# Sandy4321/dist-svgd

Measured on AMD Instinct MI355X. Metric: SVGD particle-updates/sec (n=65536,d=256) at 1/2/4/8 GPUs + % MFMA/HBM roofline, higher is better.
Workload: dtype f32; 1 GPU; dist-logreg DistSampler all_scores, Jacobi, median bandwidth; n=65536, d=256, N_global=16384, parallelism=dp1, particles_per_gpu=65536

## Files before the change

### dist-svgd_amd/csrc/phi_w1.hpp

```cpp
#pragma once
#include "gemm_x3.hpp"

namespace dsvgd {

struct PhiW1 {
  static constexpr int kThreads = 256;
  static constexpr int BM = 128, BC = 512, BJ = 16, P = 2;
  static constexpr int SA = P * BM * 32;
  static constexpr int kSmemBytes = 2 * SA;
  static constexpr int kScrLd = 44;
  static constexpr int kScrBytes = 16 * kScrLd * 4;
};

constexpr int kW1Sgb = 4;
__device__ __forceinline__ f32x4 w1_load(__amdgpu_buffer_rsrc_t r, int voff, int soff) {
  return __builtin_bit_cast(f32x4, __builtin_amdgcn_raw_buffer_load_b128(r, voff, soff, 0));
}
__device__ __forceinline__ f32x4 w1_load_nt(__amdgpu_buffer_rsrc_t r, int voff, int soff) {
  return __builtin_bit_cast(f32x4, __builtin_amdgcn_raw_buffer_load_b128(r, voff, soff, 2));
}

constexpr int w1_waves(int NI, bool EXP) { return NI == 2 && EXP ? 2 : 1; }
template <int DS, int NI = 4, bool EXP = true, int FAM = kFamRBF, class... PW>
__global__ __launch_bounds__(256)
__attribute__((amdgpu_waves_per_eu(w1_waves(NI, EXP), w1_waves(NI, EXP)))) void phi_w1_kernel(
    const float* A, int64_t a_npad, const _Float16* Yx, int64_t ldy,
    int64_t K, int64_t kchunk, const dsvgd_select_state* __restrict__ st, float* __restrict__ C,
    int64_t ldc, float* __restrict__ rowsum, int64_t m, int64_t row0, int sym,
    const float* __restrict__ colinv, int slice0, const float* __restrict__ gate, int gate_on,
    int ks_begin = 0, int ks_wrap = 0, int tcol0 = 0, int t_per = 0, int t_first = 0,
    int t_nblk = 1, int64_t t_ostride = 0, PW... pw_) {
  static_assert(sizeof...(PW) == (FAM == kFamIMQ ? 1 : 0), "pw: the IMQ instantiations only");
  [[maybe_unused]] const float pw = (0.f + ... + pw_);
  static_assert(NI == 4 || NI == 2, "NI: 4 or 2 column tiles per wave");
  static_assert(EXP || DS == 0, "the identity form is DS 0 only");
  const bool want_rs = EXP || rowsum != nullptr;
  if (gate && ((*gate != 0.f) != (gate_on != 0))) return;
  using F = FmtH2;
  constexpr int BC = 4 * 32 * NI;
  using V8 = F::V8;
  constexpr int P = PhiW1::P;
  constexpr bool TRK = DS == 1 || DS == 3 || DS == 4;
  __shared__ __attribute__((aligned(16))) char smem[PhiW1::kSmemBytes + (TRK ? 4 * PhiW1::kScrBytes : 0)];
  const int t = threadIdx.x, lane = t & 63, r = lane & 31, h = lane >> 5;
  const int w = __builtin_amdgcn_readfirstlane(t >> 6);
  const int64_t lin = (int64_t)blockIdx.z * gridDim.y + blockIdx.y;
  const bool xm = ((DS == 4 || DS == 0) && t_per == 1) || (DS == 3 && t_per > 0 && tcol0 == 1);
  const int64_t lid = lin * gridDim.x + blockIdx.x;
  const int64_t xu = (lid >> 3) * (8 / gridDim.z) + (lid & 7) / gridDim.z;
  const int64_t cbx = xm ? xu % gridDim.x : blockIdx.x;
  const int64_t by = xm ? xu / gridDim.x
                   : DS == 2 ? lin / gridDim.z
                   : DS == 1 ? (int64_t)gridDim.y - 1 - lin / gridDim.z : blockIdx.y;
  const int64_t bz = xm ? (lid & 7) % gridDim.z
                   : (DS == 1 || DS == 2) ? lin % gridDim.z : blockIdx.z;
  const bool tb = DS == 3 && t_per > 0;
  const int64_t tpart = tb ? by / t_per : 0;
  const int64_t byl = tb ? by % t_per : by;
  const int64_t i0 = byl * PhiW1::BM;
  const int64_t c0 = cbx * BC + w * 32 * NI;
  const int64_t kb0 = bz * kchunk, kend = min(K, kb0 + kchunk);
  int ks0 = (int)(kb0 / PhiW1::BJ) + (DS == 0 ? ks_begin : 0);
  int nsteps = kend > kb0 ? (int)((kend - kb0) / PhiW1::BJ) : 0;
  const int Z = (int)gridDim.z;
  const int kdir = DS == 2 ? -Z : DS == 1 ? Z : 1;
  auto wrapk = [&](int ks) { return (DS == 0 && ks_wrap > 0 && ks >= ks_wrap) ? ks - ks_wrap : ks; };
  const int kyoff = DS == 3 ? ks_begin : 0;
  if (DS == 2) {
    const int T = (int)((K - i0) / PhiW1::BJ);
    ks0 = (int)(K / PhiW1::BJ) - 1 - (int)bz;
    nsteps = T > bz ? (T - (int)bz + Z - 1) / Z : 0;
  } else if (DS == 1) {
    const int T = (int)(i0 / PhiW1::BJ);
    ks0 = (int)bz;
    nsteps = T > bz ? (T - (int)bz + Z - 1) / Z : 0;
  }
  const int ksp = DS == 4 ? (int)min(max(kb0, i0), kend) / PhiW1::BJ : 0;
  if (tb) {
    const int64_t at = ((int64_t)bz * (gridDim.y / t_per) + tpart) * t_ostride;
    C += at;
    rowsum += at;
  } else {
    C += (int64_t)(slice0 + bz) * m * ldc;
    rowsum += (int64_t)(slice0 + bz) * roundup128(m);
  }
  const float scale = !EXP ? 0.f : FAM == kFamIMQ ? st->inv_h : -st->inv_h * kLog2e;

  const __amdgpu_buffer_rsrc_t rD = __builtin_amdgcn_make_buffer_rsrc(
      (void*)(A + (i0 >> 7) * (a_npad >> 4) * kPanelElems), (short)0, 0x7fffffff, 0x00020000);
  const __amdgpu_buffer_rsrc_t rB =
      __builtin_amdgcn_make_buffer_rsrc((void*)(Yx + c0 * 16), (short)0, 0x7fffffff, 0x00020000);
  const int pstride = (int)(ldy * 32);
  const int vB = x3_off(r, h);
  const int vD = t * 32;
  const int srow = t >> 1, shalf = t & 1;
  const int aoff = x3_off(srow, shalf);
  auto diag0 = [&](int kfirst) {
    int64_t dg = row0 + i0 + srow - 8 * shalf - (int64_t)kfirst * PhiW1::BJ;
    if (DS == 0 && ks_wrap > 0 && row0 + i0 + srow < (int64_t)ks_begin * PhiW1::BJ)
      dg += (int64_t)ks_wrap * PhiW1::BJ;
    return (int)max(min(dg, (int64_t)(1 << 30)), (int64_t)-(1 << 30));
  };

  f32x16 acc[4][NI];
#pragma unroll
  for (int mi = 0; mi < 4; ++mi)
#pragma unroll
    for (int ni = 0; ni < NI; ++ni)
#pragma unroll
      for (int q = 0; q < 16; ++q) acc[mi][ni][q] = 0.f;
  float rs = 0.f;

  const int symI = tb ? (int)(((t_first + tpart) % t_nblk) * t_per + byl)
                   : DS == 3 ? tcol0 + (int)by : (sym || DS == 4) ? (int)(i0 >> 7) : -1;
  const int64_t pcols = a_npad >> 4;
  const int vP = (t >> 5) * kPanelElems * 4 + (t & 31) * 32;
  float* const scr = reinterpret_cast<float*>(smem + PhiW1::kSmemBytes + w * PhiW1::kScrBytes);
  const int sw_off = ((lane & 31) >> 1) * PhiW1::kScrLd + 16 * (lane >> 5) + 8 * (lane & 1);
  const int sr_off = 8 * shalf * PhiW1::kScrLd + (lane >> 1);

  auto phase = [&](auto TR_, const int ks0, const int nsteps, const int qd0) {
    constexpr bool TR = decltype(TR_)::value;
    if (nsteps <= 0) return;
    V8 b[NI][P];
    f32x4 dr[4][2];
    f32x4 tr[2];
    const int last = nsteps - 1;
    auto loadB = [&](int ni, int k) {
      const int soff = (wrapk(ks0 + kdir * min(k, last)) + kyoff) * P * pstride;
#pragma unroll
      for (int p = 0; p < P; ++p)
        b[ni][p] = __builtin_bit_cast(V8, w1_load(rB, vB + ni * 1024, soff + p * pstride));
    };
    auto loadD = [&](f32x4 (&d)[2], int k) {
      const int kc = min(k, last);
      const int64_t j0 = (int64_t)wrapk(ks0 + kdir * kc) * PhiW1::BJ;
      if constexpr (TR) {
        const float* src = A + (((j0 >> 7) * pcols + symI * 8) * kPanelElems + (j0 & 127) * 16);
        const __amdgpu_buffer_rsrc_t rT =
            __builtin_amdgcn_make_buffer_rsrc((void*)src, (short)0, 0x7fffffff, 0x00020000);
        d[0] = w1_load_nt(rT, vP, 0);
        d[1] = w1_load_nt(rT, vP + 16, 0);
      } else {
        const int soff = (int)(j0 >> 4) * kPanelElems * 4;
        d[0] = w1_load_nt(rD, vD, soff);
        d[1] = w1_load_nt(rD, vD + 16, soff);
      }
    };
    auto transpose = [&](const f32x4 (&d)[2], f32x4 (&o)[2]) {
      *reinterpret_cast<f32x4*>(scr + sw_off) = d[0];
      *reinterpret_cast<f32x4*>(scr + sw_off + 4) = d[1];
#pragma unroll
      for (int q = 0; q < 8; ++q) o[q >> 2][q & 3] = scr[sr_off + q * PhiW1::kScrLd];
    };
    auto stage = [&](char* st_, const f32x4 (&d)[2], int k) {
      const int qd = max(min(qd0 - kdir * k * PhiW1::BJ, 8), -1);
      float e[8];
#pragma unroll
      for (int q = 0; q < 8; ++q) {
        const float v = q < 4 ? d[0][q] : d[1][q - 4];
        const float x = !EXP ? v * F::kAScale
                        : FAM == kFamIMQ ? imq_pow(v, scale, pw, F::kAScaleLog2)
                                         : __builtin_amdgcn_exp2f(fmaf(v, scale, F::kAScaleLog2));
        e[q] = (EXP && !TR && qd == q) ? 0.f : x;
      }
      const float s = ((e[0] + e[1]) + (e[2] + e[3])) + ((e[4] + e[5]) + (e[6] + e[7]));
      rs += k <= last ? s : 0.f;
      V8 p0, p1;
#pragma unroll
      for (int q = 0; q < 8; ++q) {
        const _Float16 a0 = (_Float16)e[q];
        p0[q] = a0;
        p1[q] = (_Float16)(e[q] - (float)a0);
      }
      *reinterpret_cast<V8*>(st_ + aoff) = p0;
      *reinterpret_cast<V8*>(st_ + PhiW1::BM * 32 + aoff) = p1;
    };
    auto barrier = []() { asm volatile("s_waitcnt lgkmcnt(0)\n\ts_barrier" ::: "memory"); };
    auto step = [&](int k, const char* cur, char* nxt, const f32x4 (&ds_)[2], f32x4 (&dl)[2],
                    const f32x4 (&dt)[2]) {
      V8 a[4][P];
#pragma unroll
      for (int mi = 0; mi < 4; ++mi)
#pragma unroll
        for (int p = 0; p < P; ++p)
          a[mi][p] = *reinterpret_cast<const V8*>(cur + p * PhiW1::BM * 32 + x3_off(mi * 32 + r, h));
      if constexpr (TR)
        stage(nxt, tr, k + 1);
      else
        stage(nxt, ds_, k + 1);
#pragma unroll
      for (int ni = 0; ni < NI; ++ni) {
#pragma unroll
        for (int mi = 0; mi < 4; ++mi) acc[mi][ni] = mfma_fmt<F>(a[mi][1], b[ni][0], acc[mi][ni]);
#pragma unroll
        for (int mi = 0; mi < 4; ++mi) acc[mi][ni] = mfma_fmt<F>(a[mi][0], b[ni][1], acc[mi][ni]);
#pragma unroll
        for (int mi = 0; mi < 4; ++mi) acc[mi][ni] = mfma_fmt<F>(a[mi][0], b[ni][0], acc[mi][ni]);
        loadB(ni, k + 1);
      }
      if constexpr (TR) transpose(dt, tr);
      __builtin_amdgcn_sched_group_barrier(0x100, 8, 0);
#pragma unroll
      for (int i = 0; i < 4 * NI; ++i) {
        __builtin_amdgcn_sched_group_barrier(0x008, 1, 0);
        __builtin_amdgcn_sched_group_barrier(0x002, kW1Sgb, 0);
      }
      __builtin_amdgcn_sched_group_barrier(0x200, 2, 0);
#pragma unroll
      for (int i = 0; i < 8 * NI; ++i) {
        __builtin_amdgcn_sched_group_barrier(0x008, 1, 0);
        if (TR && i == 1) __builtin_amdgcn_sched_group_barrier(0x200, 2, 0);
        if (TR && i >= 2 && i < 10) __builtin_amdgcn_sched_group_barrier(0x100, 1, 0);
        if (i % 4 == 3) __builtin_amdgcn_sched_group_barrier(0x020, 1, 0);
      }
      loadD(dl, k + 3);
    };

#pragma unroll
    for (int ni = 0; ni < NI; ++ni) loadB(ni, 0);
    loadD(dr[0], 0);
    loadD(dr[1], 1);
    loadD(dr[2], 2);
    if constexpr (TR) {
      transpose(dr[0], tr);
      stage(smem, tr, 0);
      transpose(dr[1], tr);
    } else {
      stage(smem, dr[0], 0);
    }
    barrier();
    for (int k = 0; k < nsteps; k += 8) {
      step(k, smem, smem + PhiW1::SA, dr[1], dr[3], dr[2]);
      barrier();
      if (k + 1 >= nsteps) break;
      step(k + 1, smem + PhiW1::SA, smem, dr[2], dr[0], dr[3]);
      barrier();
      if (k + 2 >= nsteps) break;
      step(k + 2, smem, smem + PhiW1::SA, dr[3], dr[1], dr[0]);
      barrier();
      if (k + 3 >= nsteps) break;
      step(k + 3, smem + PhiW1::SA, smem, dr[0], dr[2], dr[1]);
      barrier();
      if (k + 4 >= nsteps) break;
      step(k + 4, smem, smem + PhiW1::SA, dr[1], dr[3], dr[2]);
      barrier();
      if (k + 5 >= nsteps) break;
      step(k + 5, smem + PhiW1::SA, smem, dr[2], dr[0], dr[3]);
      barrier();
      if (k + 6 >= nsteps) break;
      step(k + 6, smem, smem + PhiW1::SA, dr[3], dr[1], dr[0]);
      barrier();
      if (k + 7 >= nsteps) break;
      step(k + 7, smem + PhiW1::SA, smem, dr[0], dr[2], dr[1]);
      barrier();
    }
  };
  if constexpr (DS == 4) {
    phase(std::true_type{}, ks0, ksp - ks0, 0);
    phase(std::false_type{}, ksp, ks0 + nsteps - ksp, diag0(ksp));
  } else {
    phase(std::integral_constant<bool, DS == 1 || DS == 3>{}, ks0, nsteps, diag0(ks0));
  }

#pragma unroll
  for (int mi = 0; mi < 4; ++mi)
#pragma unroll
    for (int ni = 0; ni < NI; ++ni) {
      const int64_t col = c0 + ni * 32 + r;
      const float cs = colinv[col] * (1.f / F::kAScale);
#pragma unroll
      for (int q = 0; q < 16; ++q) {
        const int64_t row = i0 + mi * 32 + c_row(q, lane);
        if (row < m) C[row * ldc + col] = acc[mi][ni][q] * cs;
      }
    }
  {
    const float v = rs + __shfl_xor(rs, 1, 64);
    if (want_rs && cbx == 0 && shalf == 0 && i0 + srow < m)
      rowsum[i0 + srow] = v * (1.f / F::kAScale);
  }
}

}
```

Measured before the change: 4.817 million particle-updates/s.

## Split W1 K-loop into diagonal and plain phases, reschedule MFMA interleave

Splits the non-transposed K-loop into three phases so the per-element diagonal-zeroing check runs only on steps that overlap the diagonal block. Off-diagonal steps skip that compare. The change also rewrites the sched_group_barrier interleave into one loop that mixes in transcendental ops for the 2-wave variant, and simplifies the transposed-load address math with a precomputed base and scalar offsets. It disables packed-fp32 ops for the kernel. The extra phase instantiations increase code size and register pressure, and the diagonal-range math is a new source of correctness risk.

```diff
diff --git a/dist-svgd_amd/csrc/phi_w1.hpp b/dist-svgd_amd/csrc/phi_w1.hpp
--- a/dist-svgd_amd/csrc/phi_w1.hpp
+++ b/dist-svgd_amd/csrc/phi_w1.hpp
@@ -13,6 +13,8 @@
 };
 
 constexpr int kW1Sgb = 4;
+constexpr int kW1Mfv = 16;
+constexpr int kW1Exp = 8;
 __device__ __forceinline__ f32x4 w1_load(__amdgpu_buffer_rsrc_t r, int voff, int soff) {
   return __builtin_bit_cast(f32x4, __builtin_amdgcn_raw_buffer_load_b128(r, voff, soff, 0));
 }
@@ -21,6 +23,9 @@
 }
 
 constexpr int w1_waves(int NI, bool EXP) { return NI == 2 && EXP ? 2 : 1; }
+#if defined(__HIP_DEVICE_COMPILE__)
+#pragma clang attribute push(__attribute__((target("no-packed-fp32-ops"))), apply_to = function)
+#endif
 template <int DS, int NI = 4, bool EXP = true, int FAM = kFamRBF, class... PW>
 __global__ __launch_bounds__(256)
 __attribute__((amdgpu_waves_per_eu(w1_waves(NI, EXP), w1_waves(NI, EXP)))) void phi_w1_kernel(
@@ -75,7 +80,7 @@
     ks0 = (int)bz;
     nsteps = T > bz ? (T - (int)bz + Z - 1) / Z : 0;
   }
-  const int ksp = DS == 4 ? (int)min(max(kb0, i0), kend) / PhiW1::BJ : 0;
+  const int ksp = DS == 4 ? max((int)min(max(kb0, i0), kend) / PhiW1::BJ, ks0) : 0;
   if (tb) {
     const int64_t at = ((int64_t)bz * (gridDim.y / t_per) + tpart) * t_ostride;
     C += at;
@@ -119,8 +124,15 @@
   const int sw_off = ((lane & 31) >> 1) * PhiW1::kScrLd + 16 * (lane >> 5) + 8 * (lane & 1);
   const int sr_off = 8 * shalf * PhiW1::kScrLd + (lane >> 1);
 
-  auto phase = [&](auto TR_, const int ks0, const int nsteps, const int qd0) {
+  const char* const tbase = reinterpret_cast<const char*>(A + (int64_t)symI * 8 * kPanelElems);
+  const uint32_t trow = (uint32_t)(pcols * kPanelElems * 4);
+
+  auto phase = [&](auto TR_, auto DG_, auto U_, const int ks0, const int nsteps,
+                   const int qd0) __attribute__((always_inline)) {
     constexpr bool TR = decltype(TR_)::value;
+    constexpr bool DG = decltype(DG_)::value;
+    constexpr int U = decltype(U_)::value;
+    static_assert(!(TR && DG) && (U == 4 || U == 8), "phase: TR or DG; 4 or 8 K-steps per trip");
     if (nsteps <= 0) return;
     V8 b[NI][P];
     f32x4 dr[4][2];
@@ -133,16 +145,15 @@
         b[ni][p] = __builtin_bit_cast(V8, w1_load(rB, vB + ni * 1024, soff + p * pstride));
     };
     auto loadD = [&](f32x4 (&d)[2], int k) {
-      const int kc = min(k, last);
-      const int64_t j0 = (int64_t)wrapk(ks0 + kdir * kc) * PhiW1::BJ;
+      const int ks = wrapk(ks0 + kdir * min(k, last));
       if constexpr (TR) {
-        const float* src = A + (((j0 >> 7) * pcols + symI * 8) * kPanelElems + (j0 & 127) * 16);
-        const __amdgpu_buffer_rsrc_t rT =
-            __builtin_amdgcn_make_buffer_rsrc((void*)src, (short)0, 0x7fffffff, 0x00020000);
-        d[0] = w1_load_nt(rT, vP, 0);
-        d[1] = w1_load_nt(rT, vP + 16, 0);
+        const __amdgpu_buffer_rsrc_t rT = __builtin_amdgcn_make_buffer_rsrc(
+            (void*)(tbase + (uint64_t)(uint32_t)(ks >> 3) * trow), (short)0, 0x7fffffff, 0x00020000);
+        const int soff = (ks & 7) * (PhiW1::BJ * 16 * 4);
+        d[0] = w1_load_nt(rT, vP, soff);
+        d[1] = w1_load_nt(rT, vP + 16, soff);
       } else {
-        const int soff = (int)(j0 >> 4) * kPanelElems * 4;
+        const int soff = ks * kPanelElems * 4;
         d[0] = w1_load_nt(rD, vD, soff);
         d[1] = w1_load_nt(rD, vD + 16, soff);
       }
@@ -154,7 +165,7 @@
       for (int q = 0; q < 8; ++q) o[q >> 2][q & 3] = scr[sr_off + q * PhiW1::kScrLd];
     };
     auto stage = [&](char* st_, const f32x4 (&d)[2], int k) {
-      const int qd = max(min(qd0 - kdir * k * PhiW1::BJ, 8), -1);
+      [[maybe_unused]] const int qd = DG ? max(min(qd0 - kdir * k * PhiW1::BJ, 8), -1) : -1;
       float e[8];
 #pragma unroll
       for (int q = 0; q < 8; ++q) {
@@ -162,7 +173,7 @@
         const float x = !EXP ? v * F::kAScale
                         : FAM == kFamIMQ ? imq_pow(v, scale, pw, F::kAScaleLog2)
                                          : __builtin_amdgcn_exp2f(fmaf(v, scale, F::kAScaleLog2));
-        e[q] = (EXP && !TR && qd == q) ? 0.f : x;
+        e[q] = (EXP && DG && qd == q) ? 0.f : x;
       }
       const float s = ((e[0] + e[1]) + (e[2] + e[3])) + ((e[4] + e[5]) + (e[6] + e[7]));
       rs += k <= last ? s : 0.f;
@@ -200,19 +211,18 @@
         loadB(ni, k + 1);
       }
       if constexpr (TR) transpose(dt, tr);
+      constexpr int kTrReads = NI == 4 ? 8 : 4;
       __builtin_amdgcn_sched_group_barrier(0x100, 8, 0);
 #pragma unroll
-      for (int i = 0; i < 4 * NI; ++i) {
+      for (int i = 0; i < 12 * NI; ++i) {
         __builtin_amdgcn_sched_group_barrier(0x008, 1, 0);
-        __builtin_amdgcn_sched_group_barrier(0x002, kW1Sgb, 0);
-      }
-      __builtin_amdgcn_sched_group_barrier(0x200, 2, 0);
-#pragma unroll
-      for (int i = 0; i < 8 * NI; ++i) {
-        __builtin_amdgcn_sched_group_barrier(0x008, 1, 0);
-        if (TR && i == 1) __builtin_amdgcn_sched_group_barrier(0x200, 2, 0);
-        if (TR && i >= 2 && i < 10) __builtin_amdgcn_sched_group_barrier(0x100, 1, 0);
-        if (i % 4 == 3) __builtin_amdgcn_sched_group_barrier(0x020, 1, 0);
+        if (NI == 2 && EXP && i < kW1Exp) __builtin_amdgcn_sched_group_barrier(0x400, 1, 0);
+        if (i < kW1Mfv) __builtin_amdgcn_sched_group_barrier(0x002, kW1Sgb, 0);
+        if (i == kW1Mfv - 1) __builtin_amdgcn_sched_group_barrier(0x200, 2, 0);
+        if (TR && i == kW1Mfv + 1) __builtin_amdgcn_sched_group_barrier(0x200, 2, 0);
+        if (TR && i >= kW1Mfv + 2 && i < kW1Mfv + 2 + kTrReads)
+          __builtin_amdgcn_sched_group_barrier(0x100, 1, 0);
+        if (i >= 4 * NI && i % 4 == 3) __builtin_amdgcn_sched_group_barrier(0x020, 1, 0);
       }
       loadD(dl, k + 3);
     };
@@ -230,7 +240,7 @@
       stage(smem, dr[0], 0);
     }
     barrier();
-    for (int k = 0; k < nsteps; k += 8) {
+    for (int k = 0; k < nsteps; k += U) {
       step(k, smem, smem + PhiW1::SA, dr[1], dr[3], dr[2]);
       barrier();
       if (k + 1 >= nsteps) break;
@@ -242,25 +252,47 @@
       if (k + 3 >= nsteps) break;
       step(k + 3, smem + PhiW1::SA, smem, dr[0], dr[2], dr[1]);
       barrier();
-      if (k + 4 >= nsteps) break;
-      step(k + 4, smem, smem + PhiW1::SA, dr[1], dr[3], dr[2]);
-      barrier();
-      if (k + 5 >= nsteps) break;
-      step(k + 5, smem + PhiW1::SA, smem, dr[2], dr[0], dr[3]);
-      barrier();
-      if (k + 6 >= nsteps) break;
-      step(k + 6, smem, smem + PhiW1::SA, dr[3], dr[1], dr[0]);
-      barrier();
-      if (k + 7 >= nsteps) break;
-      step(k + 7, smem + PhiW1::SA, smem, dr[0], dr[2], dr[1]);
-      barrier();
+      if constexpr (U == 8) {
+        if (k + 4 >= nsteps) break;
+        step(k + 4, smem, smem + PhiW1::SA, dr[1], dr[3], dr[2]);
+        barrier();
+        if (k + 5 >= nsteps) break;
+        step(k + 5, smem + PhiW1::SA, smem, dr[2], dr[0], dr[3]);
+        barrier();
+        if (k + 6 >= nsteps) break;
+        step(k + 6, smem, smem + PhiW1::SA, dr[3], dr[1], dr[0]);
+        barrier();
+        if (k + 7 >= nsteps) break;
+        step(k + 7, smem + PhiW1::SA, smem, dr[0], dr[2], dr[1]);
+        barrier();
+      }
     }
   };
+  using C8 = std::integral_constant<int, 8>;
+  auto plain = [&](const int kbase, const int n) {
+    const int dlo = (int)((row0 + i0) >> 4), dhi = (int)((row0 + i0 + PhiW1::BM - 1) >> 4);
+    int ka, kb;
+    if constexpr (DS == 2) {
+      ka = min((max(kbase - dhi, 0) + Z - 1) / Z, n);
+      kb = kbase < dlo ? ka : max(min((kbase - dlo) / Z + 1, n), ka);
+    } else {
+      ka = min(max(dlo - kbase, 0), n);
+      kb = max(min(dhi + 1 - kbase, n), ka);
+    }
+    if (DS == 0 && ks_wrap > 0) ka = 0, kb = n;
+    if constexpr (DS != 4) phase(std::false_type{}, std::false_type{}, C8{}, kbase, ka, 0);
+    phase(std::false_type{}, std::true_type{}, std::integral_constant<int, DS == 0 ? 8 : 4>{},
+          kbase + kdir * ka, kb - ka, diag0(kbase + kdir * ka));
+    phase(std::false_type{}, std::false_type{}, C8{}, kbase + kdir * kb, n - kb, 0);
+  };
   if constexpr (DS == 4) {
-    phase(std::true_type{}, ks0, ksp - ks0, 0);
-    phase(std::false_type{}, ksp, ks0 + nsteps - ksp, diag0(ksp));
+    phase(std::true_type{}, std::false_type{}, C8{}, ks0, ksp - ks0, 0);
+    plain(ksp, ks0 + nsteps - ksp);
+  } else if constexpr (DS == 1 || DS == 3 || !EXP) {
+    phase(std::integral_constant<bool, DS == 1 || DS == 3>{}, std::false_type{}, C8{}, ks0, nsteps,
+          0);
   } else {
-    phase(std::integral_constant<bool, DS == 1 || DS == 3>{}, ks0, nsteps, diag0(ks0));
+    plain(ks0, nsteps);
   }
 
 #pragma unroll
@@ -281,5 +313,8 @@
       rowsum[i0 + srow] = v * (1.f / F::kAScale);
   }
 }
+#if defined(__HIP_DEVICE_COMPILE__)
+#pragma clang attribute pop
+#endif
 
 }
```

Result: no change. 4.838 million particle-updates/s, median of 6 (+0.4%).
